# wwu98934/MuRCL

Measured on AMD Instinct MI355X. Metric: WSI-bags/sec pretrain step (ABMIL+NT-Xent) at N=2048,d=512, higher is better.
Workload: dtype bf16

## Files before the change

### include/murcl_amd.h

```cpp
#ifndef MURCL_AMD_H
#define MURCL_AMD_H
#include <stdint.h>
#ifdef __cplusplus
extern "C" {
#endif

typedef struct ihipStream_t* murcl_stream_t;

#define MURCL_F32 0
#define MURCL_BF16 1

#define MURCL_EPI_NONE 0
#define MURCL_EPI_BIAS 1
#define MURCL_EPI_BIAS_RELU 2
#define MURCL_EPI_MASK 3
#define MURCL_EPI_RANK1_MASK 4

int murcl_gemm_nt(const void* A, const void* B, void* C, int M, int N, int K, int lda, int ldb, int ldc,
                  int dtype_in, int dtype_out, int epilogue, const float* bias, const void* mask, int ldmask,
                  const float* rowscale, const float* rank1, int rows_per_bag, float* colsum_ws, int accumulate,
                  murcl_stream_t stream);

typedef struct murcl_tn_problem {
    const void* A; const void* B; float* C;
    const float* colsum_part; float* colsum_out;
    int M, N1, N2, lda, ldb, ldc, colsum_rows;
    int flags;
    float scale;
} murcl_tn_problem;
#define MURCL_TN_OVERWRITE 1
#define MURCL_TN_DEINTERLEAVE 2
#define MURCL_TN_SCALE 4
#define MURCL_TN_KIND_EMPTY 0
#define MURCL_TN_KIND_SMALL 1
#define MURCL_TN_KIND_SQUARE 2
#define MURCL_TN_KIND_PARTS 3
#define MURCL_TN_KIND_ATOMIC 4
#define MURCL_TN_KIND_WIDE 5
#define MURCL_TN_MAXG 4
long murcl_gemm_tn_plan(const murcl_tn_problem* probs, int n, int dtype, int* kinds);
int murcl_gemm_tn_grouped(const murcl_tn_problem* probs, int n, int dtype, float* ws, long ws_bytes, murcl_stream_t stream);

int murcl_panel_gemm_supported(int M, int N, int K, int epilogue, int rows_per_bag);
int murcl_panel_gemm_colsum_rows(int M, int N, int K, int epilogue);
int murcl_panel_gemm(const void* A, const void* W, void* C, int M, int N, int K, int epilogue, const float* bias,
                     void* bitmask_out, const void* bitmask_in, const float* rowscale, const float* rank1,
                     int rows_per_bag, float* colsum_out, int colsum_accumulate, float* colsum_ws ,
                     int walk_reverse, murcl_stream_t stream);
int murcl_panel_gemm_drop(const void* A, const void* W, void* C, int M, int N, int K, int epilogue, const float* bias,
                          void* bitmask_out, const void* bitmask_in, const float* rowscale, const float* rank1,
                          int rows_per_bag, float* colsum_out, int colsum_accumulate, float* colsum_ws, int walk_reverse,
                          float keep_p, unsigned long long seed_a, unsigned long long seed_b, murcl_stream_t stream);

int murcl_cu_budget(void);
int murcl_set_cu_budget(int cus);

int murcl_calib_copy(const void* src, void* dst, long bytes, murcl_stream_t stream);
int murcl_calib_mfma_bf16(float* out_256x512, int iters, murcl_stream_t stream);

int murcl_abmil_pool_workspace(int B, int N, int dtype, int* chunk_rows, int* n_chunks);
int murcl_abmil_pool_fwd(const void* H, const void* Wa, const float* ba, const float* wb, const float* bb,
                         float* scores, float* A, float* M, float* ml, float* part_ws, int B, int N, int L, int D,
                         int dtype, int exact_tanh, murcl_stream_t stream);
int murcl_abmil_pool_combine(const float* scores, const float* part_ws, float* A, float* M, float* ml, int B, int N,
                             int dtype, murcl_stream_t stream);
// ... 181 lines not shown
```

### murcl_amd/_lib.py

```python
import ctypes
import os

import torch

_HERE = os.path.dirname(os.path.abspath(__file__))
LIB_PATH = os.environ.get("MURCL_AMD_LIB") or os.path.join(_HERE, "libmurcl_amd.so")

F32, BF16 = 0, 1
EPI_NONE, EPI_BIAS, EPI_BIAS_RELU, EPI_MASK, EPI_RANK1_MASK = 0, 1, 2, 3, 4

_c = ctypes
_P, _I, _L, _F = _c.c_void_p, _c.c_int, _c.c_long, _c.c_float

SIGNATURES = {
    "murcl_gemm_nt": [_P, _P, _P, _I, _I, _I, _I, _I, _I, _I, _I, _I, _P, _P, _I, _P, _P, _I, _P, _I, _P],
    "murcl_gemm_tn_plan": [_P, _I, _I, _P],
    "murcl_gemm_tn_grouped": [_P, _I, _I, _P, _L, _P],
    "murcl_panel_gemm_colsum_rows": [_I, _I, _I, _I],
    "murcl_panel_gemm_supported": [_I, _I, _I, _I, _I],
    "murcl_panel_gemm": [_P, _P, _P, _I, _I, _I, _I, _P, _P, _P, _P, _P, _I, _P, _I, _P, _I, _P],
    "murcl_panel_gemm_drop": [_P, _P, _P, _I, _I, _I, _I, _P, _P, _P, _P, _P, _I, _P, _I, _P, _I, _F, ctypes.c_ulonglong, ctypes.c_ulonglong, _P],
    "murcl_cu_budget": [],
    "murcl_set_cu_budget": [_I],
    "murcl_calib_copy": [_P, _P, _L, _P],
# ... 69 lines not shown
    "murcl_gru_step_supported": [_I, _I, _I],
    "murcl_gru_step_fwd": [_P, _P, _I, _P, _P, _P, _P, _P, _P, _P, _I, _I, _P],
    "murcl_gru_step_bwd": [_P, _P, _P, _P, _P, _P, _P, _P, _P, _I, _I, _I, _I, _P],
    "murcl_ppo_act_workspace": [_I, _I, _I],
    "murcl_ppo_act": [_P, _I, _I, _I, _P, _P, _P, _F, _I, _P, _P, _P, _P, _P],
    "murcl_ppo_epoch_workspace": [_I, _I, _I, _I],
    "murcl_ppo_epoch": [_P, _P, _I, _I, _I, _P, _P, _P, _P, _I, _I, _L, _F, _F, _F, _P, _P, _P],
    "murcl_ppo_epoch_wt": [_P, _P, _P, _I, _I, _I, _P, _P, _P, _P, _I, _I, _L, _F, _F, _F, _P, _P, _P],
    "murcl_step_draws": [ctypes.c_ulonglong, _P, _L, _P, _L, _P, _P, _I, _I, _F, _P],
    "murcl_stack_lists": [_P, _I, _P],
    "murcl_add_lists": [_P, _I, _P],
    "murcl_cast_batch": [_P, _I, _I, _P],
    "murcl_cast_batch_flat": [_P, _P, _I, _I, _P],
    "murcl_cast_batch_flat_tick": [_P, _P, _I, _I, _P, _P],
    "murcl_relu_bitmask": [_P, _P, _I, _I, _I, _I, _P],
    "murcl_dropout_relu_bitmask": [_P, _P, _I, _I, _F, _F, ctypes.c_ulonglong, _I, _P],
    "murcl_adam_step": [_P, _P, _P, _P, _L, _F, _F, _F, _F, _F, _I, _I, _P],
    "murcl_adam_multi": [_P, _I, _F, _F, _F, _F, _I, _P],
    "murcl_adam_multi_live": [_P, _I, _F, _F, _F, _F, _I, _P, _P],
    "murcl_adam_multi_live_deferred": [_P, _I, _F, _F, _F, _F, _I, _P, _P],
    "murcl_replay_tick": [_P, _P],
    "murcl_sgd_step": [_P, _P, _P, _L, _F, _F, _I, _F, _I, _I, _P],
}
_RESTYPE = {"murcl_ntxent_workspace_bytes": _L, "murcl_ntxent_xchg_bytes": _L, "murcl_kmeans_workspace_bytes": _L, "murcl_ppo_act_workspace": _L, "murcl_gemm_tn_plan": _L,
            "murcl_ppo_epoch_workspace": _L}



class TnProblem(ctypes.Structure):
    _fields_ = [("A", _P), ("B", _P), ("C", _P), ("colsum_part", _P), ("colsum_out", _P),
                ("M", _I), ("N1", _I), ("N2", _I), ("lda", _I), ("ldb", _I), ("ldc", _I), ("colsum_rows", _I), ("flags", _I), ("scale", _F)]


TN_OVERWRITE, TN_DEINTERLEAVE, TN_SCALE = 1, 2, 4
TN_KIND_EMPTY, TN_KIND_SMALL, TN_KIND_SQUARE, TN_KIND_PARTS, TN_KIND_ATOMIC, TN_KIND_WIDE = 0, 1, 2, 3, 4, 5
TN_MAXG = 4


_lib = None


def lib():
    global _lib
    if _lib is None:
        if not os.path.exists(LIB_PATH):
            raise RuntimeError(
                f"{LIB_PATH} not found: build it with `python -m murcl_amd.build` "
                "(murcl_amd has no CPU/PyTorch fallback for its kernels)")
        L = ctypes.CDLL(LIB_PATH)
        for name, args in SIGNATURES.items():
            fn = getattr(L, name)
            fn.argtypes = args
            fn.restype = _RESTYPE.get(name, _I)
        _lib = L
    return _lib


def check(rc, what):
    if rc != 0:
        raise RuntimeError(f"murcl_amd: {what} failed with code {rc}")


def ptr(t):
    return None if t is None else t.data_ptr()


_raw_stream = getattr(torch._C, "_cuda_getCurrentRawStream", None)
# ... 15 lines not shown
```

### murcl_amd/csrc/gemm.hip

```cpp
#include "common.h"

enum { EPI_NONE = 0, EPI_BIAS = 1, EPI_BIAS_RELU = 2, EPI_MASK = 3, EPI_RANK1_MASK = 4 };

struct GemmEpi {
    const float* bias;
    const void* mask;
    int ldmask;
    const float* rowscale;
    const float* rank1;
    int rows_per_bag;
    float* colsum_ws;
    int accumulate;
};

template <typename T> struct Frag;
template <> struct Frag<bf16_t> { typedef bf16x8 type; };
template <> struct Frag<float> { typedef f32x4 type; };

template <typename T>
__device__ __forceinline__ f32x4 mma16(typename Frag<T>::type a, typename Frag<T>::type b, f32x4 c);
template <>
__device__ __forceinline__ f32x4 mma16<bf16_t>(bf16x8 a, bf16x8 b, f32x4 c) {
    return __builtin_amdgcn_mfma_f32_16x16x32_bf16(a, b, c, 0, 0, 0);
}
// ... 918 lines not shown
            __builtin_amdgcn_sched_group_barrier(0x008, NJ / 4, 0);
            __builtin_amdgcn_sched_group_barrier(0x100, 1, 0);
            __builtin_amdgcn_sched_group_barrier(0x008, NJ / 4, 0);
            __builtin_amdgcn_sched_group_barrier(0x100, 1, 0);
            __builtin_amdgcn_sched_group_barrier(0x008, NJ / 2, 0);
        }
        __builtin_amdgcn_sched_group_barrier(0x008, 2 * NJ, 0);
    }
    float* pt = part + (size_t)sp * N1 * N2;
    const int q4 = lane >> 4, r16 = lane & 15;
#pragma unroll
    for (int i = 0; i < 8; ++i)
#pragma unroll
        for (int j = 0; j < NJ; ++j) {
            const int n2 = n20 + wc * (16 * NJ) + j * 16 + r16;
#pragma unroll
            for (int r = 0; r < 4; ++r) {
                const int n1 = n10 + wr * 128 + i * 16 + 4 * q4 + r;
                pt[(size_t)n1 * N2 + n2] = acc[i][j][r];
            }
        }
}
struct TnReduceArgs {
    float* C[TN_MAXG];
    const float* cs_part[TN_MAXG];
    float* cs_out[TN_MAXG];
    long part_off[TN_MAXG], n4[TN_MAXG];
    int nsplit[TN_MAXG], N1[TN_MAXG], N2[TN_MAXG], ldc[TN_MAXG], cs_rows[TN_MAXG], flags[TN_MAXG];
    float scale[TN_MAXG];
    int blk0[TN_MAXG + 1];
    int cs_blk0[TN_MAXG + 1];
    int n;
};
__global__ __launch_bounds__(256) void tn_reduce_kernel(const float* __restrict__ ws, const TnReduceArgs ra) {
    int blk = blockIdx.x;
    if (blk >= ra.blk0[ra.n]) {
        blk -= ra.blk0[ra.n];
        int g = 0;
        while (g + 1 < ra.n && blk >= ra.cs_blk0[g + 1]) ++g;
        blk -= ra.cs_blk0[g];
        const float* __restrict__ cs_part = ra.cs_part[g];
        if (cs_part == nullptr) return;
        const int cs_rows = ra.cs_rows[g];
        __shared__ f32x4 red[256];
        const int cg = threadIdx.x & 15, rs = threadIdx.x >> 4;
        const long j = (long)blk * 16 + cg;
        const int ng = ra.N1[g] / 4;
        f32x4 b0 = {0, 0, 0, 0}, b1 = b0;
        if (j < ng) {
            const f32x4* q = (const f32x4*)cs_part + j;
            for (int r0 = 0; r0 < cs_rows; r0 += 256) {
                f32x4 v[16];
#pragma unroll
                for (int k = 0; k < 16; ++k) {
                    const int r = r0 + rs + 16 * k;
                    v[k] = r < cs_rows ? q[(size_t)r * ng] : f32x4{0, 0, 0, 0};
                }
#pragma unroll
                for (int k = 0; k < 16; k += 2) { b0 += v[k]; b1 += v[k + 1]; }
            }
        }
        red[threadIdx.x] = b0 + b1;
        __syncthreads();
        if (rs == 0 && j < ng) {
            f32x4 t = red[cg];
#pragma unroll
            for (int k = 1; k < 16; ++k) t += red[16 * k + cg];
            if (ra.flags[g] & MURCL_TN_SCALE) t *= ra.scale[g];
            f32x4* o = (f32x4*)ra.cs_out[g] + j;
            *o = (ra.flags[g] & MURCL_TN_OVERWRITE) ? t : *o + t;
        }
        return;
    }
    int g = 0;
    while (g + 1 < ra.n && blk >= ra.blk0[g + 1]) ++g;
    const long i = (long)(blk - ra.blk0[g]) * 256 + threadIdx.x;
    const long n4 = ra.n4[g];
    if (i >= n4) return;
    const int nsplit = ra.nsplit[g], N2 = ra.N2[g];
    const f32x4* p = (const f32x4*)(ws + ra.part_off[g]) + i;
    f32x4 a0 = {0, 0, 0, 0}, a1 = a0, a2 = a0, a3 = a0;
    int s = 0;
    for (; s + 3 < nsplit; s += 4) {
        const f32x4 v0 = p[(size_t)s * n4], v1 = p[(size_t)(s + 1) * n4], v2 = p[(size_t)(s + 2) * n4], v3 = p[(size_t)(s + 3) * n4];
        a0 += v0; a1 += v1; a2 += v2; a3 += v3;
    }
    for (; s < nsplit; ++s) a0 += p[(size_t)s * n4];
    f32x4 t = (a0 + a1) + (a2 + a3);
    const int fl = ra.flags[g];
    if (fl & MURCL_TN_SCALE) t *= ra.scale[g];
    const long e = i * 4, col = e % N2;
    long row = e / N2;
    if (fl & MURCL_TN_DEINTERLEAVE) row = ((row >> 4) & 1) * (ra.N1[g] >> 1) + (row >> 5) * 16 + (row & 15);
    f32x4* c = (f32x4*)(ra.C[g] + row * ra.ldc[g] + col);
    *c = (fl & MURCL_TN_OVERWRITE) ? t : *c + t;
}
static bool tn_sq_ok(int M, int N1, int N2, int ldc, int dtype) {
    return dtype == MURCL_DTYPE_BF16 && N1 % 256 == 0 && N2 % 256 == 0 && M >= 16384 && ldc % 4 == 0;
}
struct TnPlan { int sp[TN_MAXG], mps[TN_MAXG], tiles[TN_MAXG]; long part_off[TN_MAXG]; long ws_floats; int wgs; };
static bool tn_group_plan(int n, const int* M, const int* N1, const int* N2, TnPlan* pl, unsigned* map) {
    if (n < 1 || n > TN_MAXG) return false;
    long work = 0;
    int pairs = 0;
    for (int g = 0; g < n; ++g) {
        pl->tiles[g] = (N1[g] / 256) * (N2[g] / 256);
        if (pl->tiles[g] > murcl_cu_budget() / 8) return false;
        work += (long)pl->tiles[g] * M[g];
        pairs += pl->tiles[g];
    }
    const int cap = murcl_cu_budget();
    if (pairs > cap) return false;
    long R = ((work + cap - 1) / cap + 31) / 32 * 32;
    if (R < 8 * 32) R = 8 * 32;
    for (;; R += ((R >> 8) + 31) / 32 * 32) {
        int total = 0;
        for (int g = 0; g < n; ++g) {
            pl->sp[g] = (int)((M[g] + R - 1) / R);
            total += pl->sp[g] * pl->tiles[g];
        }
        if (total <= cap) { pl->wgs = total; break; }
    }
    long off = 0;
    for (int g = 0; g < n; ++g) {
        long mps = ((M[g] + pl->sp[g] - 1) / pl->sp[g] + 31) / 32 * 32;
        pl->mps[g] = (int)mps;
        pl->sp[g] = (int)((M[g] + mps - 1) / mps);
        pl->part_off[g] = off;
// ... 68 lines not shown
        if (mc & 15) {
            const int nz = (mp - mc) * 32;
            for (int i = tid; i < 2 * nz; i += 256) {
                const int which = i >= nz, j = which ? i - nz : i;
                *(float*)(ts_smem + (which ? slab_b : 0u) + (mc * 32 + j) * 4) = 0.f;
            }
            __syncthreads();
        }
        const char* la = ts_smem + aoff;
        const char* lb = ts_smem + slab_b + boff;
        for (int u = 0; u < mp / 16; ++u) {
            f32x4 a, b;
#pragma unroll
            for (int e = 0; e < 4; ++e) {
                a[e] = *(const float*)(la + (16 * u + 4 * e) * 128);
                b[e] = *(const float*)(lb + (16 * u + 4 * e) * 128);
            }
            if (u & 1) acc1 = mma16<float>(a, b, acc1); else acc0 = mma16<float>(a, b, acc0);
            if (do_cs) accs = mma16<float>(a, f32x4{1.f, 1.f, 1.f, 1.f}, accs);
        }
    }
    const int n2 = n20 + 16 * wn + r16;
#pragma unroll
    for (int r = 0; r < 4; ++r) {
        const int n1 = n10 + 16 * wm + 4 * q4 + r;
        if (n1 < N1 && n2 < N2) C[(size_t)n1 * ldc + n2] = cold[r] + (acc0[r] + acc1[r]);
        if (do_cs && r16 == 0 && n1 < N1) colsum_out[n1] = overwrite ? accs[r] : colsum_out[n1] + accs[r];
    }
}
struct TnSmallGroup {
    const float* A[4]; const float* B[4]; float* C[4]; float* cs[4];
    int M[4], N1[4], N2[4], lda[4], ldb[4], ldc[4], tile0[5], pass_rows, overwrite[4];
};
__global__ __launch_bounds__(256) void gemm_tn_small_group_kernel(const TnSmallGroup ga) {
    extern __shared__ __attribute__((aligned(16))) char ts_smem[];
    const int b = blockIdx.x;
    int g = 0;
#pragma unroll
    for (int i = 1; i < 4; ++i) g += (int)(b >= ga.tile0[i]);
    const int t = b - ga.tile0[g], t1 = (ga.N1[g] + TS_T - 1) / TS_T;
    tn_small_tile(ga.A[g], ga.B[g], ga.C[g], ga.M[g], ga.N1[g], ga.N2[g], ga.lda[g], ga.ldb[g], ga.ldc[g], ga.cs[g], t % t1, t / t1,
                  ts_smem, ga.pass_rows, ga.overwrite[g]);
}
static int tn_small_pass_rows(int M, long tiles) {
    int pr = TS_MAXM;
    if (tiles > 512 && M > 192) pr = ((M + 1) / 2 + 15) & ~15;
    pr = (pr + 15) & ~15;
    if (pr > TS_MAXM) pr = TS_MAXM;
    if (pr < 16) pr = 16;
    return pr;
}


static void tn_generic_plan(int M, int N1, int N2, int dtype, bool x3, int& splits, int& mps) {
    const int rows = dtype == MURCL_DTYPE_BF16 ? 64 : 32;
    const int t1 = (N1 + 127) / 128, t2 = (N2 + 127) / 128;
    if (M <= 8 * rows && (long)N1 * N2 >= (1L << 20)) {
        splits = 1;
    } else {
        const int target = (dtype == MURCL_DTYPE_F32 && !x3 && M >= 16384) ? 2 * murcl_cu_budget() : murcl_cu_budget();
        splits = (target + t1 * t2 - 1) / (t1 * t2);
        if (splits >= 8) splits = ((splits + 7) / 8) * 8;
        if (murcl_cu_budget() < 256 && splits >= 8)
            while (splits > 8 && splits * t1 * t2 > target) splits -= 8;
        while (splits > 8 && (long)(splits - 8) * rows * 4 >= M) splits -= 8;
        while (splits > 1 && splits < 8 && (long)(splits - 1) * rows * 4 >= M) --splits;
    }
    mps = (M + splits - 1) / splits;
    mps = ((mps + rows - 1) / rows) * rows;
    if ((long)mps * (splits - 1) >= M) splits = (M + mps - 1) / mps;
}

constexpr int TN_PARTS_MIN_M = 16384;
static_assert(TN_MAXG == MURCL_TN_MAXG, "include/murcl_amd.h");

typedef murcl_tn_problem TnProblem;
struct TnStep { int kind, splits, mps; long ws_bytes; };

static int tn_plan_one(const TnProblem& p, int dtype, TnStep& st) {
    st = TnStep{MURCL_TN_KIND_EMPTY, 0, 0, 0};
    if (p.M <= 0 || p.N1 <= 0 || p.N2 <= 0) return p.flags ? -1 : 0;
    if (p.colsum_part && (!p.colsum_out || p.colsum_rows <= 0 || p.N1 % 4)) return -1;
    const bool x3 = dtype == MURCL_DTYPE_F32X3;
    const int base = x3 ? MURCL_DTYPE_F32 : dtype;
    if (base != MURCL_DTYPE_F32 && base != MURCL_DTYPE_BF16) return -1;
    const int es = base == MURCL_DTYPE_BF16 ? 2 : 4, epc = 16 / es;
    if (p.N1 < epc || p.N2 < epc || p.N1 % epc || p.N2 % epc || (p.lda * es) % 16 || (p.ldb * es) % 16) return -1;
    TnPlan pl;
    if (tn_sq_ok(p.M, p.N1, p.N2, p.ldc, dtype) && tn_group_plan(1, &p.M, &p.N1, &p.N2, &pl, nullptr)) {
        st = TnStep{MURCL_TN_KIND_SQUARE, pl.sp[0], pl.mps[0], pl.ws_floats * 4};
        return p.flags && p.colsum_out && !p.colsum_part ? -1 : 0;
    }
    if (dtype == MURCL_DTYPE_BF16 && p.N1 % 256 == 0 && p.N2 % 128 == 0 && p.M >= 4096) {
        const int tiles = (p.N1 / 256) * (p.N2 / 128);
        int sp = (256 + tiles - 1) / tiles;
        sp = ((sp + 7) / 8) * 8;
        while (sp > 8 && (long)(sp - 8) * 64 * 4 >= p.M) sp -= 8;
        int mps = (p.M + sp - 1) / sp;
        mps = ((mps + 63) / 64) * 64;
        if ((long)mps * (sp - 1) >= p.M) sp = (p.M + mps - 1) / mps;
        st = TnStep{MURCL_TN_KIND_WIDE, sp, mps, 0};
        return p.flags ? -1 : 0;
    }
    if (dtype == MURCL_DTYPE_F32 && p.M <= TS_MAXM) {
        st = TnStep{MURCL_TN_KIND_SMALL, 1, p.M, 0};
        return (p.flags & ~MURCL_TN_OVERWRITE) || (p.flags && p.colsum_part) ? -1 : 0;
    }
    int splits, mps;
    tn_generic_plan(p.M, p.N1, p.N2, base, x3, splits, mps);
    if (p.M >= TN_PARTS_MIN_M && splits > 1 && (long)mps * (splits - 1) < p.M)
        st = TnStep{MURCL_TN_KIND_PARTS, splits, mps, (long)splits * ((long)p.N1 * p.N2 + p.N1) * 4};
    else
        st = TnStep{MURCL_TN_KIND_ATOMIC, splits, mps, 0};
    return p.flags ? -1 : 0;
}

enum { TN_EACH, TN_SMALL_GROUP, TN_SQ_GROUP };
static long tn_plan(const TnProblem* pr, int n, int dtype, int* kinds, int& form) {
    form = TN_EACH;
    bool small = n <= TN_MAXG, sq = n <= TN_MAXG;
    long ws = 0;
    int M[TN_MAXG], N1[TN_MAXG], N2[TN_MAXG];
    for (int g = 0; g < n; ++g) {
        TnStep st;
        if (tn_plan_one(pr[g], dtype, st)) return -1;
        if (kinds) kinds[g] = st.kind;
        small = small && st.kind == MURCL_TN_KIND_SMALL && !pr[g].colsum_part;
        sq = sq && st.kind == MURCL_TN_KIND_SQUARE;
        ws = st.ws_bytes > ws ? st.ws_bytes : ws;
        if (g < TN_MAXG) { M[g] = pr[g].M; N1[g] = pr[g].N1; N2[g] = pr[g].N2; }
    }
    if (n < 1) return 0;
    if (small) form = TN_SMALL_GROUP;
    TnPlan pl;
    if (sq && tn_group_plan(n, M, N1, N2, &pl, nullptr)) {
        form = TN_SQ_GROUP;
        ws = pl.ws_floats * 4;
    }
    return ws;
}

extern "C" long murcl_gemm_tn_plan(const TnProblem* pr, int n, int dtype, int* kinds) {
    int form;
    return tn_plan(pr, n, dtype, kinds, form);
}

static int tn_small_launch(const TnProblem* pr, int n, hipStream_t stream) {
    TnSmallGroup ga;
    int tiles = 0, mmax = 0;
    for (int g = 0; g < 4; ++g) {
        const TnProblem& p = pr[g < n ? g : 0];
        ga.A[g] = (const float*)p.A; ga.B[g] = (const float*)p.B; ga.C[g] = p.C; ga.cs[g] = p.colsum_out;
        ga.M[g] = p.M; ga.N1[g] = p.N1; ga.N2[g] = p.N2; ga.lda[g] = p.lda; ga.ldb[g] = p.ldb; ga.ldc[g] = p.ldc;
        ga.overwrite[g] = (p.flags & MURCL_TN_OVERWRITE) ? 1 : 0;
        ga.tile0[g] = tiles;
        if (g < n) {
            tiles += ((p.N1 + TS_T - 1) / TS_T) * ((p.N2 + TS_T - 1) / TS_T);
            if (p.M > mmax) mmax = p.M;
        }
    }
    for (int g = n; g < 5; ++g) ga.tile0[g] = tiles;
    ga.pass_rows = tn_small_pass_rows(mmax, tiles);
    const int mp = ((mmax < ga.pass_rows ? mmax : ga.pass_rows) + 15) & ~15;
    static MurclOncePerDevice once;
    if (once.first())
        hipFuncSetAttribute((const void*)gemm_tn_small_group_kernel, hipFuncAttributeMaxDynamicSharedMemorySize, 2 * TS_MAXM * 128);
    hipLaunchKernelGGL(gemm_tn_small_group_kernel, dim3(tiles), dim3(256), 2 * mp * 128, stream, ga);
    return MURCL_CHECK_LAUNCH();
}

static int tn_sq_launch(const TnProblem* pr, int n, int dtype, float* ws, hipStream_t stream) {
    int M[TN_MAXG], N1[TN_MAXG], N2[TN_MAXG];
    for (int g = 0; g < n; ++g) {
        M[g] = pr[g].M; N1[g] = pr[g].N1; N2[g] = pr[g].N2;
        if (pr[g].colsum_out && !pr[g].colsum_part) {
            const int rc = murcl_colsum(pr[g].A, pr[g].colsum_out, pr[g].M, pr[g].N1, pr[g].lda, dtype, 1, stream);
            if (rc) return rc;
        }
    }
    TnPlan pl;
    TnGroupArgs ga;
    if (!tn_group_plan(n, M, N1, N2, &pl, ga.map)) return -1;
    TnReduceArgs ra;
    ra.n = n;
    int blk = 0, csb = 0;
    for (int g = 0; g < TN_MAXG; ++g) {
        const int h = g < n ? g : 0;
        ga.A[g] = (const bf16_t*)pr[h].A; ga.B[g] = (const bf16_t*)pr[h].B;
        ga.M[g] = pr[h].M; ga.N1[g] = pr[h].N1; ga.N2[g] = pr[h].N2; ga.lda[g] = pr[h].lda; ga.ldb[g] = pr[h].ldb;
        ga.mps[g] = pl.mps[h]; ga.part_off[g] = pl.part_off[h];
        ra.C[g] = pr[h].C; ra.cs_part[g] = pr[h].colsum_part; ra.cs_out[g] = pr[h].colsum_part ? pr[h].colsum_out : nullptr;
        ra.cs_rows[g] = pr[h].colsum_rows;
        ra.part_off[g] = pl.part_off[h]; ra.n4[g] = (long)pr[h].N1 * pr[h].N2 / 4; ra.nsplit[g] = pl.sp[h];
        ra.N1[g] = pr[h].N1; ra.N2[g] = pr[h].N2; ra.ldc[g] = pr[h].ldc; ra.flags[g] = pr[h].flags; ra.scale[g] = pr[h].scale;
        if (g < n) {
            ra.blk0[g] = blk; blk += (int)((ra.n4[g] + 255) / 256);
            ra.cs_blk0[g] = csb; csb += pr[g].colsum_part ? (pr[g].N1 / 4 + 15) / 16 : 0;
        }
    }
    for (int g = n; g <= TN_MAXG; ++g) { ra.blk0[g] = blk; ra.cs_blk0[g] = csb; }
    auto k = gemm_tn_sq_kernel<TN_SQ_WAVES>;
    constexpr int LDS = TN_SQ_NSLOT * 32768;
    static MurclOncePerDevice once;
    if (once.first()) { hipFuncSetAttribute((const void*)k, hipFuncAttributeMaxDynamicSharedMemorySize, LDS); }
    hipLaunchKernelGGL(k, dim3(TN_MAXWG), dim3(64 * TN_SQ_WAVES), LDS, stream, ga, ws);
    int rc = MURCL_CHECK_LAUNCH();
    if (rc) return rc;
    hipLaunchKernelGGL(tn_reduce_kernel, dim3((unsigned)(blk + csb)), dim3(256), 0, stream, (const float*)ws, ra);
    return MURCL_CHECK_LAUNCH();
}

static int tn_launch_one(TnProblem p, int dtype, float* ws, hipStream_t stream) {
    TnStep st;
    tn_plan_one(p, dtype, st);
    if (st.kind == MURCL_TN_KIND_EMPTY) return 0;
    if (st.kind == MURCL_TN_KIND_SQUARE) return tn_sq_launch(&p, 1, dtype, ws, stream);
    if (p.colsum_part) {
        const int rc = murcl_colsum(p.colsum_part, p.colsum_out, p.colsum_rows, p.N1, p.N1, MURCL_DTYPE_F32, 1, stream);
        if (rc) return rc;
        p.colsum_out = nullptr;
    }
    if (st.kind == MURCL_TN_KIND_SMALL) return tn_small_launch(&p, 1, stream);
    const void *A = p.A, *B = p.B;
    float *C = p.C, *colsum_out = p.colsum_out;
    const int M = p.M, N1 = p.N1, N2 = p.N2, lda = p.lda, ldb = p.ldb, ldc = p.ldc, splits = st.splits, mps = st.mps;
    if (st.kind == MURCL_TN_KIND_WIDE) {
        if (colsum_out) {
            const int rc = murcl_colsum(A, colsum_out, M, N1, lda, dtype, 1, stream);
            if (rc) return rc;
        }
        auto k = gemm_tn_wide_kernel;
        constexpr int LDS = 3 * 49152;
        static MurclOncePerDevice once;
        if (once.first()) { hipFuncSetAttribute((const void*)k, hipFuncAttributeMaxDynamicSharedMemorySize, LDS); }
        hipLaunchKernelGGL(k, dim3((N1 / 256) * (N2 / 128) * splits), dim3(512), LDS, stream, (const bf16_t*)A, (const bf16_t*)B, C,
                           M, N1, N2, lda, ldb, ldc, mps, splits);
        return MURCL_CHECK_LAUNCH();
    }
    const bool x3 = dtype == MURCL_DTYPE_F32X3;
    float* part = st.kind == MURCL_TN_KIND_PARTS ? ws : nullptr;
    const int rows = dtype == MURCL_DTYPE_BF16 ? 64 : 32;
    const int t1 = (N1 + 127) / 128, t2 = (N2 + 127) / 128;
    dim3 grid(t1 * t2 * splits);
    const bool deep = (t1 * t2 * splits <= 256 || splits == 1) && mps > rows;
#define TN_LAUNCH(T, NS, X3)                                                                                        \
    {                                                                                                               \
        auto k = gemm_tn_kernel<T, NS, X3>;                                                                         \
        static MurclOncePerDevice once;                                                                                         \
        if (once.first()) { hipFuncSetAttribute((const void*)k, hipFuncAttributeMaxDynamicSharedMemorySize, NS * 32768); } \
        hipLaunchKernelGGL(k, grid, dim3(256), NS * 32768, stream, (const T*)A, (const T*)B, C, M, N1, N2, lda, ldb, ldc, mps, \
                           splits, colsum_out, part);                                                               \
    }
    if (dtype == MURCL_DTYPE_BF16) {
        if (deep) TN_LAUNCH(bf16_t, 4, false) else TN_LAUNCH(bf16_t, 2, false)
    } else if (x3) {
        if (deep) TN_LAUNCH(float, 4, true) else TN_LAUNCH(float, 2, true)
    } else {
        if (deep) TN_LAUNCH(float, 4, false) else TN_LAUNCH(float, 2, false)
    }
#undef TN_LAUNCH
    if (part) {
        const int rc = MURCL_CHECK_LAUNCH();
        if (rc) return rc;
        const long n = (long)N1 * N2 + (colsum_out ? N1 : 0);
        hipLaunchKernelGGL(tn_split_reduce_kernel, dim3((unsigned)((n + 31) / 32)), dim3(256), 0, stream, part, C, colsum_out, N1, N2,
                           ldc, splits);
    }
    return MURCL_CHECK_LAUNCH();
}

extern "C" int murcl_gemm_tn_grouped(const TnProblem* pr, int n, int dtype, float* ws, long ws_bytes, hipStream_t stream) {
    int form;
    const long need = tn_plan(pr, n, dtype, nullptr, form);
    if (need < 0 || (need > 0 && (!ws || ws_bytes < need))) return -1;
    if (form == TN_SMALL_GROUP) return tn_small_launch(pr, n, stream);
    if (form == TN_SQ_GROUP) return tn_sq_launch(pr, n, dtype, ws, stream);
    for (int g = 0; g < n; ++g) {
        const int rc = tn_launch_one(pr[g], dtype, ws, stream);
        if (rc) return rc;
    }
    return 0;
}
```

### murcl_amd/functional.py

```python
import math

import torch

from . import ops


def _flat2(x):
    return x.reshape(-1, x.shape[-1])


_DIRECT = False


def set_direct_grad(flag):
    global _DIRECT
    _DIRECT = bool(flag)


_MILESTONE = None
_STREAM_A = 4
_FUSED_GATE = True
_GATE_U = True
_FUSED_FC_DROP = True
_FUSED_INST = True
_DSMIL_REASSOC = True
_DSMIL_ONEPASS = True
_DSMIL_QV = True
_DSMIL_X3 = True
_GROUP_WGRAD = True
_FOLD_BIAS = True
_FRAG_WEIGHTS = True


def _frag_specs(w1, w2, w3, wa, T):
    return [(w1, False, T, "frag"), (w2, False, T, "frag"), (w3, False, T, "frag"), (wa, False, T, "frag"),
            (wa, True, T), (w3, True, T, "frag"), (w2, True, T, "frag")]


_OVERLAP_BUDGET = None


def set_overlap_cu_budget(cus):
    global _OVERLAP_BUDGET
    _OVERLAP_BUDGET = None if cus is None else int(cus)


class _overlap_budget:

    def __enter__(self):
        self.prev = None
        if _OVERLAP_BUDGET is not None:
            self.prev = ops.cu_budget()
            ops.set_cu_budget(min(self.prev, _OVERLAP_BUDGET))
        return self

    def __exit__(self, *exc):
        if self.prev is not None:
            ops.set_cu_budget(self.prev)
        return False


def set_grad_milestone(callback):
    global _MILESTONE
    _MILESTONE = callback
# ... 73 lines not shown
def _wgrad_group(items):
    probs = []
    for dy, x, w, b, parts in items:
        if _direct(w):
            probs.append((dy, x, w.grad, b.grad.view(-1) if parts is not None else None, parts))
            _touch(w)
            if parts is not None:
                _touch(b)
        else:
            assert parts is None
            probs.append((dy, x, None, None, None))
    Cs = ops.gemm_tn_grouped(probs, fresh=True)
    return [None if _direct(it[2]) else C for it, C in zip(items, Cs)]


_DEFERRED = None
_DEFER_ON = True


class deferred_wgrads:
    def __enter__(self):
        global _DEFERRED
        self.prev, _DEFERRED = _DEFERRED, ({} if _DEFER_ON else None)
        return self

    def __exit__(self, *exc):
        global _DEFERRED
        queue, _DEFERRED = _DEFERRED, self.prev
        if exc[0] is None and queue:
            _flush(queue)
        return False


def _flush(queue):
    probs = []
    for w, b, dys, xs in queue.values():
        dy = dys[0] if len(dys) == 1 else torch.cat(dys, 0)
        x = xs[0] if len(xs) == 1 else torch.cat(xs, 0)
        probs.append((dy, x, w.grad, b.grad.view(-1) if b is not None else None, None))
    queue.clear()
    for i in range(0, len(probs), 4):
        ops.gemm_tn_grouped(probs[i:i + 4])


def flush_deferred():
    if _DEFERRED:
        _flush(_DEFERRED)


def _defer(dy, x, w, b):
    if _DEFERRED is None or not _direct(w) or (b is not None and not _direct(b)):
        return False
    ent = _DEFERRED.get(id(w))
    if ent is None:
        ent = _DEFERRED[id(w)] = (w, b, [], [])
    elif (ent[1] is None) != (b is None):
        return False
    ent[2].append(dy)
    ent[3].append(x)
    _touch(w, b)
    return True


def _wbgrad(dy, x, w, b):
    if _defer(dy, x, w, b):
        return None, None
    if _direct(w) and _direct(b):
        ops.gemm_tn(dy, x, out=w.grad, colsum_into=b.grad.view(-1))
        _touch(w, b)
        return None, None
    return _wgrad(dy, x, w), _bgrad(dy, b)


def _bgrad(dy, b):
    if _direct(b):
# ... 155 lines not shown
        if m3 is not None:
            dT, dba, dwb, dbb = ops.abmil_pool_bwd(h3.view(B, N, L), wac, ba, wb, scores, ml, M, dM, into=into_k2, frag=wfrag)
        else:
            dT, dba, dwb, dbb, A = ops.abmil_pool_bwd(h3.view(B, N, L), wac, ba, wb, scores, ml, M, dM, into=into_k2, want_A=True,
                                                      frag=wfrag)
        dwa = _wgrad(dT, h3, wa)
        if direct_k2:
            _touch(ba, wb, bb)
            _final(wa, ba, wb, bb, wd, bd)
        if m3 is not None:
            def into(b):
                if _direct(b):
                    _touch(b)
                    return b.grad.view(-1)
                return None
            fold = lambda w, b: _FOLD_BIAS and _direct(w) and _direct(b)
            f3, f2, f1 = fold(w3, b3), fold(w2, b2), fold(w1, b1)
            grouped = _GROUP_WGRAD and _MILESTONE is None
            dz3, _, db3 = ops.panel_gemm(dT, wat, ops.PG_RANK1_MASK, bitmask=m3, rowscale=scores.view(-1), bias=ml, rank1=dM,
                                         rows_per_bag=N, colsum=True, colsum_into=None if f3 else into(b3), colsum_defer=f3,
                                         frag=False)
            if not grouped:
                dw3 = _wgrad(dz3, h2, w3, b3, db3 if f3 else None)
                _final(w3, b3)
            dz2, _, db2 = ops.panel_gemm(dz3, w3t, ops.PG_MASK, bitmask=m2, colsum=True,
                                         colsum_into=None if f2 else into(b2), colsum_defer=f2, frag=wfrag)
            if not grouped:
                dw2 = _wgrad(dz2, h1, w2, b2, db2 if f2 else None)
                _final(w2, b2)
            dz1, _, db1 = ops.panel_gemm(dz2, w2t, ops.PG_MASK, bitmask=m1, colsum=True,
                                         colsum_into=None if f1 else into(b1), colsum_defer=f1, frag=wfrag)
            budget_scope.__exit__()
            if grouped:
                dw3, dw2, dw1 = _wgrad_group([(dz3, h2, w3, b3, db3 if f3 else None), (dz2, h1, w2, b2, db2 if f2 else None),
                                              (dz1, x2, w1, b1, db1 if f1 else None)])
                _final(w3, b3, w2, b2, w1, b1)
            db3, db2 = None if f3 else db3, None if f2 else db2
            if grouped:
                db1 = None if f1 else db1
        else:
            dz3, ws = ops.gemm_nt(dT, wat, epi=ops.EPI_RANK1_MASK, mask=h3, rowscale=A.view(-1),
                                  rank1=dM, rows_per_bag=N, colsum=True)
            db3 = _bgrad(ws, b3)
            dw3 = _wgrad(dz3, h2, w3)
            _final(w3, b3)
            dz2, ws = ops.gemm_nt(dz3, w3t, epi=ops.EPI_MASK, mask=h2, colsum=True)
            db2 = _bgrad(ws, b2)
            dw2 = _wgrad(dz2, h1, w2)
            _final(w2, b2)
            dz1, ws = ops.gemm_nt(dz2, w2t, epi=ops.EPI_MASK, mask=h1, colsum=True)
            db1 = _bgrad(ws, b1)
            budget_scope.__exit__()
        if m3 is not None and grouped:
            pass
        elif m3 is not None and f1:
            dw1, db1 = _wgrad(dz1, x2, w1, b1, db1), None
        else:
            dw1 = _wgrad(dz1, x2, w1)
        dx = None
        if need_dx:
            dx = ops.gemm_nt(dz1, ops.transpose_cast(w1, T)).view(B, N, d)
        if direct_k2:
            dba = dwb = dbb = None
        else:
            dba, dwb, dbb = _pgrad(dba, ba), _pgrad(dwb.reshape(1, -1), wb), _pgrad(dbb, bb)
        return dx, dw1, db1, dw2, db2, dw3, db3, dwa, dba, dwb, dbb, dwd, dbd

    @staticmethod
# ... 861 lines not shown
```

### murcl_amd/ops.py

```python
import ctypes
import math

import torch

from . import _lib
from ._lib import BF16, F32, EPI_BIAS, EPI_BIAS_RELU, EPI_MASK, EPI_NONE, EPI_RANK1_MASK, check, dt, ptr, stream

_TORCH_DT = {F32: torch.float32, BF16: torch.bfloat16}
_EPI_NAME = {EPI_NONE: "NONE", EPI_BIAS: "BIAS", EPI_BIAS_RELU: "BIAS_RELU", EPI_MASK: "MASK", EPI_RANK1_MASK: "RANK1_MASK"}
_DT_NAME = {torch.float32: "f32", torch.bfloat16: "bf16"}


class KernelTimers:

    def __init__(self, only=None, every=1, pool=0):
        self.only, self.every, self.records, self._seen = only, max(1, int(every)), {}, {}
        self._pool = [torch.cuda.Event(enable_timing=True) for _ in range(int(pool))]

    def event(self):
        return self._pool.pop() if self._pool else torch.cuda.Event(enable_timing=True)

    def span(self, key, work=None):
        if self.only is not None and key not in self.only:
            return _NULL
# ... 202 lines not shown
            check(_lib.lib().murcl_panel_gemm_drop(ptr(A), ptr(W), ptr(C), M, N, K, epi, ptr(bias), ptr(bm), ptr(bitmask),
                                                   ptr(rowscale), ptr(rank1), rows_per_bag,
                                                   ptr(colsum_into if colsum_into is not None else cs),
                                                   int(colsum_into is not None), ptr(ws), int(reverse) | (2 if stream_a else 0) | wfrag,
                                                   drop.keep_p, drop.seed, 0, stream()), "panel_gemm(drop)")
        else:
            check(_lib.lib().murcl_panel_gemm(ptr(A), ptr(W), ptr(C), M, N, K, epi, ptr(bias), ptr(bm), ptr(bitmask),
                                              ptr(rowscale), ptr(rank1), rows_per_bag,
                                              ptr(colsum_into if colsum_into is not None else cs),
                                              int(colsum_into is not None), ptr(ws), int(reverse) | (2 if stream_a else 0) | wfrag, stream()),
                  "panel_gemm")
    if colsum_defer:
        return C, bm, (ws, _lib.lib().murcl_panel_gemm_colsum_rows(M, N, K, epi))
    return C, bm, cs


def relu_bitmask(x):
    _need_cuda(x)
    x = _c(x)
    M, N = x.shape
    bits = torch.empty((M, N // 8), dtype=torch.uint8, device=x.device)
    check(_lib.lib().murcl_relu_bitmask(ptr(x), ptr(bits), M, N, N, dt(x), stream()), "relu_bitmask")
    return bits


_TN_NAME = {_lib.TN_KIND_SQUARE: "gemm_tn_sq", _lib.TN_KIND_WIDE: "gemm_tn_wide"}
_CODE_NAME = {F32: "f32", BF16: "bf16", F32X3: "f32x3"}


def gemm_tn_plan(problems, code):
    n = len(problems)
    arr, kinds = (_lib.TnProblem * n)(), (ctypes.c_int * n)()
    for g, (A, B, _, ci, cp, opts) in enumerate(problems):
        assert A.dtype == B.dtype == problems[0][0].dtype and A.shape[0] == B.shape[0]
        (M, N1), N2 = A.shape, B.shape[1]
        flags, scale = 0, 1.0
        if opts and opts.get("scale") is not None:
            flags, scale = flags | _lib.TN_SCALE, float(opts["scale"])
        if opts and opts.get("deinterleave"):
            flags |= _lib.TN_DEINTERLEAVE
        if opts and opts.get("overwrite"):
            flags |= _lib.TN_OVERWRITE
        assert ci is None or (ci.dtype == torch.float32 and ci.is_contiguous() and ci.numel() == N1)
        arr[g] = _lib.TnProblem(ptr(A), ptr(B), None, ptr(cp[0]) if cp else None, ptr(ci), M, N1, N2, N1, N2, N2, cp[1] if cp else 0,
                                flags, scale)
    return arr, _lib.lib().murcl_gemm_tn_plan(arr, n, code, kinds), list(kinds)


def _tn_sq_group(kinds):
    return 1 < len(kinds) <= _lib.TN_MAXG and all(k == _lib.TN_KIND_SQUARE for k in kinds)


def _tn_run(problems, code, plan, write):
    arr, wsb, kinds = plan
    if wsb < 0:
        raise RuntimeError(f"murcl_amd: murcl_gemm_tn_plan rejects {[(tuple(p[0].shape), tuple(p[1].shape)) for p in problems]} ({wsb})")
    Cs, written = [], False
    for g, (A, B, out, *_) in enumerate(problems):
        N1, N2 = A.shape[1], B.shape[1]
        if out is None:
            written = write(kinds[g], problems[g])
            out = (torch.empty if written else torch.zeros)((N1, N2), dtype=torch.float32, device=A.device)
            if written:
                arr[g].flags |= _lib.TN_OVERWRITE
        assert out.dtype == torch.float32 and out.is_contiguous() and tuple(out.shape) == (N1, N2)
        arr[g].C = ptr(out)
        Cs.append(out)
    ws = torch.empty((wsb // 4,), dtype=torch.float32, device=Cs[0].device) if wsb else None
    if _tn_sq_group(kinds):
        key = f"gemm_tn_sq_grouped{len(kinds)}<bf16>"
    elif all(k == _lib.TN_KIND_SMALL for k in kinds) and (len(kinds) > 1 or written):
        key = None
    else:
        key = "+".join(sorted({_TN_NAME.get(k, "gemm_tn") for k in kinds})) + f"<{_CODE_NAME[code]}>"
    span = _span(lambda: (key, dict(flops=sum(2.0 * p[0].shape[0] * p[0].shape[1] * p[1].shape[1] for p in problems),
                                    bytes=sum(p[0].shape[0] * (p[0].shape[1] + p[1].shape[1]) * p[0].element_size()
                                              + p[0].shape[1] * p[1].shape[1] * 4 for p in problems)))) if key else _NULL
    with span:
        check(_lib.lib().murcl_gemm_tn_grouped(arr, len(problems), code, ptr(ws), wsb, stream()), "gemm_tn_grouped")
    return Cs


def gemm_tn_with_colsum(A, B):
    _need_cuda(A, B)
    A, B = _c(A), _c(B)
    cs = torch.empty((A.shape[1],), dtype=torch.float32, device=A.device)
    probs = [(A, B, None, cs, None, None)]
    plan = gemm_tn_plan(probs, dt(A))
    if plan[1] < 0 or plan[2][0] != _lib.TN_KIND_SMALL:
        return gemm_tn(A, B), colsum(A)
    return _tn_run(probs, dt(A), plan, lambda k, p: True)[0], cs


def gemm_tn(A, B, *, out=None, colsum_into=None, colsum_parts=None, x3=False):
    _need_cuda(A, B)
    A, B = _c(A), _c(B)
    M, N1 = A.shape
    N2 = B.shape[1]
    assert B.shape[0] == M and A.dtype == B.dtype
    epc = 4 if A.dtype == torch.float32 else 8
    if colsum_parts is not None and (colsum_into is None or N1 % 4):
        raise ValueError("colsum_parts needs colsum_into and N1 % 4 == 0")
    if N1 % epc:
        res = gemm_tn(pad_cols(A, ((N1 + epc - 1) // epc) * epc), B)[:N1]
        if colsum_into is not None:
            colsum(A, out=colsum_into, accumulate=True)
        if out is None:
            return res.contiguous()
        if out.is_contiguous() and out.dtype == torch.float32:
            return axpby(out, res, 1.0, 1.0, out=out)
        return out.add_(res)
    fresh = out is None and colsum_into is None and not x3
    code = F32X3 if (x3 and A.dtype == torch.float32 and M >= 4096) else dt(A)
    probs = [(A, B, out, colsum_into, colsum_parts, None)]
    return _tn_run(probs, code, gemm_tn_plan(probs, code), lambda k, p: fresh and k == _lib.TN_KIND_SMALL)[0]


def gemm_tn_grouped(problems, fresh=False):
    problems = [(_c(p[0]), _c(p[1])) + tuple(p[2:]) + (None,) * (6 - len(p)) for p in problems]
    _need_cuda(*(t for p in problems for t in p[:2]))
    if any(p[0].shape[1] % (16 // p[0].element_size()) for p in problems):
        assert all(p[5] is None for p in problems), "scale / deinterleave / overwrite need the grouped launch"
        return [gemm_tn(A, B, out=out, colsum_into=ci, colsum_parts=cp) for A, B, out, ci, cp, _ in problems]
    code = dt(problems[0][0])
    plan = gemm_tn_plan(problems, code)
    sq_group = _tn_sq_group(plan[2])
    return _tn_run(problems, code, plan, lambda k, p: (k == _lib.TN_KIND_SMALL and p[3] is None)
                   or (k == _lib.TN_KIND_SQUARE and fresh and sq_group))


def gemm_tn_grouped_ok(problems):
    problems = [tuple(p) + (None,) * (6 - len(p)) for p in problems]
    _, wsb, kinds = gemm_tn_plan(problems, dt(problems[0][0]))
    return wsb >= 0 and _tn_sq_group(kinds)


def cu_budget():
    return _lib.lib().murcl_cu_budget()


def set_cu_budget(cus):
    return _lib.lib().murcl_set_cu_budget(int(cus))


def pool_chunks(B, N, dtype_code):
    cr, nc = ctypes.c_int(), ctypes.c_int()
    _lib.lib().murcl_abmil_pool_workspace(B, N, dtype_code, ctypes.byref(cr), ctypes.byref(nc))
    return cr.value, nc.value


def _pool_work(B, N, L, D, es):
    return dict(flops=B * (2.0 * N * L * D + 2.0 * N * D + 2.0 * N * L), bytes=B * (N * L * es + N * 4 + L * 4) + L * D * es)


def abmil_pool_partials(H, Wa, ba, wb, bb, exact_tanh=None, scores=None, frag=None):
    _need_cuda(H, Wa)
    wfrag = 2 if (is_frag(Wa) if frag is None else frag) else 0
    H, Wa = _c(H), (Wa if wfrag else _c(Wa))
    B, N, L = H.shape
    D = Wa.shape[0]
    if exact_tanh is None:
# ... 1033 lines not shown
```

Before: 44820.

## Fold deferred small f32 head wgrads into the square-group TN reduce launch

Adds an F32_IN flag so a grouped TN GEMM can mix bf16 square problems with f32 small problems. When the MLP wgrad group is deferred, the small head weight-gradient GEMMs are run inside the same epilogue kernel that performs the split-K reduction of the square group, instead of as separate launches. The aim is to cut kernel launches and tail idle time in the backward pass. The cost is more complex planning and the small tiles sharing a kernel with reduce blocks, with LDS sized for the larger of the two.

```diff
diff --git a/include/murcl_amd.h b/include/murcl_amd.h
--- a/include/murcl_amd.h
+++ b/include/murcl_amd.h
@@ -31,6 +31,7 @@
 #define MURCL_TN_OVERWRITE 1
 #define MURCL_TN_DEINTERLEAVE 2
 #define MURCL_TN_SCALE 4
+#define MURCL_TN_F32_IN 8
 #define MURCL_TN_KIND_EMPTY 0
 #define MURCL_TN_KIND_SMALL 1
 #define MURCL_TN_KIND_SQUARE 2
diff --git a/murcl_amd/_lib.py b/murcl_amd/_lib.py
--- a/murcl_amd/_lib.py
+++ b/murcl_amd/_lib.py
@@ -125,7 +125,7 @@
                 ("M", _I), ("N1", _I), ("N2", _I), ("lda", _I), ("ldb", _I), ("ldc", _I), ("colsum_rows", _I), ("flags", _I), ("scale", _F)]
 
 
-TN_OVERWRITE, TN_DEINTERLEAVE, TN_SCALE = 1, 2, 4
+TN_OVERWRITE, TN_DEINTERLEAVE, TN_SCALE, TN_F32_IN = 1, 2, 4, 8
 TN_KIND_EMPTY, TN_KIND_SMALL, TN_KIND_SQUARE, TN_KIND_PARTS, TN_KIND_ATOMIC, TN_KIND_WIDE = 0, 1, 2, 3, 4, 5
 TN_MAXG = 4
 
diff --git a/murcl_amd/csrc/gemm.hip b/murcl_amd/csrc/gemm.hip
--- a/murcl_amd/csrc/gemm.hip
+++ b/murcl_amd/csrc/gemm.hip
@@ -974,8 +974,7 @@
     int cs_blk0[TN_MAXG + 1];
     int n;
 };
-__global__ __launch_bounds__(256) void tn_reduce_kernel(const float* __restrict__ ws, const TnReduceArgs ra) {
-    int blk = blockIdx.x;
+__device__ __forceinline__ void tn_reduce_block(const float* __restrict__ ws, const TnReduceArgs& ra, int blk, f32x4* red) {
     if (blk >= ra.blk0[ra.n]) {
         blk -= ra.blk0[ra.n];
         int g = 0;
@@ -984,7 +983,6 @@
         const float* __restrict__ cs_part = ra.cs_part[g];
         if (cs_part == nullptr) return;
         const int cs_rows = ra.cs_rows[g];
-        __shared__ f32x4 red[256];
         const int cg = threadIdx.x & 15, rs = threadIdx.x >> 4;
         const long j = (long)blk * 16 + cg;
         const int ng = ra.N1[g] / 4;
@@ -1036,6 +1034,10 @@
     if (fl & MURCL_TN_DEINTERLEAVE) row = ((row >> 4) & 1) * (ra.N1[g] >> 1) + (row >> 5) * 16 + (row & 15);
     f32x4* c = (f32x4*)(ra.C[g] + row * ra.ldc[g] + col);
     *c = (fl & MURCL_TN_OVERWRITE) ? t : *c + t;
+}
+__global__ __launch_bounds__(256) void tn_reduce_kernel(const float* __restrict__ ws, const TnReduceArgs ra) {
+    __shared__ f32x4 red[256];
+    tn_reduce_block(ws, ra, blockIdx.x, red);
 }
 static bool tn_sq_ok(int M, int N1, int N2, int ldc, int dtype) {
     return dtype == MURCL_DTYPE_BF16 && N1 % 256 == 0 && N2 % 256 == 0 && M >= 16384 && ldc % 4 == 0;
@@ -1170,15 +1172,23 @@
     const float* A[4]; const float* B[4]; float* C[4]; float* cs[4];
     int M[4], N1[4], N2[4], lda[4], ldb[4], ldc[4], tile0[5], pass_rows, overwrite[4];
 };
-__global__ __launch_bounds__(256) void gemm_tn_small_group_kernel(const TnSmallGroup ga) {
-    extern __shared__ __attribute__((aligned(16))) char ts_smem[];
-    const int b = blockIdx.x;
+__device__ __forceinline__ void tn_small_block(const TnSmallGroup& ga, int b, char* ts_smem) {
     int g = 0;
 #pragma unroll
     for (int i = 1; i < 4; ++i) g += (int)(b >= ga.tile0[i]);
     const int t = b - ga.tile0[g], t1 = (ga.N1[g] + TS_T - 1) / TS_T;
     tn_small_tile(ga.A[g], ga.B[g], ga.C[g], ga.M[g], ga.N1[g], ga.N2[g], ga.lda[g], ga.ldb[g], ga.ldc[g], ga.cs[g], t % t1, t / t1,
                   ts_smem, ga.pass_rows, ga.overwrite[g]);
+}
+__global__ __launch_bounds__(256) void gemm_tn_small_group_kernel(const TnSmallGroup ga) {
+    extern __shared__ __attribute__((aligned(16))) char ts_smem[];
+    tn_small_block(ga, blockIdx.x, ts_smem);
+}
+__global__ __launch_bounds__(256) void tn_epilogue_kernel(const float* __restrict__ ws, const TnReduceArgs ra, const TnSmallGroup sg) {
+    extern __shared__ __attribute__((aligned(16))) char ts_smem[];
+    const int ns = sg.tile0[4];
+    if ((int)blockIdx.x < ns) tn_small_block(sg, blockIdx.x, ts_smem);
+    else tn_reduce_block(ws, ra, (int)blockIdx.x - ns, (f32x4*)ts_smem);
 }
 static int tn_small_pass_rows(int M, long tiles) {
     int pr = TS_MAXM;
@@ -1215,8 +1225,13 @@
 typedef murcl_tn_problem TnProblem;
 struct TnStep { int kind, splits, mps; long ws_bytes; };
 
-static int tn_plan_one(const TnProblem& p, int dtype, TnStep& st) {
+static int tn_plan_one(TnProblem p, int dtype, TnStep& st) {
     st = TnStep{MURCL_TN_KIND_EMPTY, 0, 0, 0};
+    if (p.flags & MURCL_TN_F32_IN) {
+        if (dtype != MURCL_DTYPE_BF16) return -1;
+        dtype = MURCL_DTYPE_F32;
+        p.flags &= ~MURCL_TN_F32_IN;
+    }
     if (p.M <= 0 || p.N1 <= 0 || p.N2 <= 0) return p.flags ? -1 : 0;
     if (p.colsum_part && (!p.colsum_out || p.colsum_rows <= 0 || p.N1 % 4)) return -1;
     const bool x3 = dtype == MURCL_DTYPE_F32X3;
@@ -1253,10 +1268,12 @@
     return p.flags ? -1 : 0;
 }
 
-enum { TN_EACH, TN_SMALL_GROUP, TN_SQ_GROUP };
-static long tn_plan(const TnProblem* pr, int n, int dtype, int* kinds, int& form) {
+enum { TN_EACH, TN_SMALL_GROUP, TN_SQ_GROUP, TN_EPILOGUE };
+static long tn_plan(const TnProblem* pr, int n, int dtype, int* kinds, int& form, int* nsq = nullptr) {
     form = TN_EACH;
+    if (nsq) *nsq = 0;
     bool small = n <= TN_MAXG, sq = n <= TN_MAXG;
+    int lead = 0, tail = 0;
     long ws = 0;
     int M[TN_MAXG], N1[TN_MAXG], N2[TN_MAXG];
     for (int g = 0; g < n; ++g) {
@@ -1265,6 +1282,8 @@
         if (kinds) kinds[g] = st.kind;
         small = small && st.kind == MURCL_TN_KIND_SMALL && !pr[g].colsum_part;
         sq = sq && st.kind == MURCL_TN_KIND_SQUARE;
+        if (st.kind == MURCL_TN_KIND_SQUARE && lead == g && lead < TN_MAXG) ++lead;
+        else if (st.kind == MURCL_TN_KIND_SMALL && !pr[g].colsum_part && (pr[g].flags & MURCL_TN_F32_IN) && lead && tail < 4) ++tail;
         ws = st.ws_bytes > ws ? st.ws_bytes : ws;
         if (g < TN_MAXG) { M[g] = pr[g].M; N1[g] = pr[g].N1; N2[g] = pr[g].N2; }
     }
@@ -1274,6 +1293,10 @@
     if (sq && tn_group_plan(n, M, N1, N2, &pl, nullptr)) {
         form = TN_SQ_GROUP;
         ws = pl.ws_floats * 4;
+    } else if (tail && lead + tail == n && tn_group_plan(lead, M, N1, N2, &pl, nullptr)) {
+        form = TN_EPILOGUE;
+        ws = pl.ws_floats * 4;
+        if (nsq) *nsq = lead;
     }
     return ws;
 }
@@ -1283,8 +1306,7 @@
     return tn_plan(pr, n, dtype, kinds, form);
 }
 
-static int tn_small_launch(const TnProblem* pr, int n, hipStream_t stream) {
-    TnSmallGroup ga;
+static int tn_small_args(const TnProblem* pr, int n, TnSmallGroup& ga, int& lds) {
     int tiles = 0, mmax = 0;
     for (int g = 0; g < 4; ++g) {
         const TnProblem& p = pr[g < n ? g : 0];
@@ -1300,14 +1322,22 @@
     for (int g = n; g < 5; ++g) ga.tile0[g] = tiles;
     ga.pass_rows = tn_small_pass_rows(mmax, tiles);
     const int mp = ((mmax < ga.pass_rows ? mmax : ga.pass_rows) + 15) & ~15;
+    lds = 2 * mp * 128;
+    return tiles;
+}
+static int tn_small_launch(const TnProblem* pr, int n, hipStream_t stream) {
+    TnSmallGroup ga;
+    int lds;
+    const int tiles = tn_small_args(pr, n, ga, lds);
     static MurclOncePerDevice once;
     if (once.first())
         hipFuncSetAttribute((const void*)gemm_tn_small_group_kernel, hipFuncAttributeMaxDynamicSharedMemorySize, 2 * TS_MAXM * 128);
-    hipLaunchKernelGGL(gemm_tn_small_group_kernel, dim3(tiles), dim3(256), 2 * mp * 128, stream, ga);
+    hipLaunchKernelGGL(gemm_tn_small_group_kernel, dim3(tiles), dim3(256), lds, stream, ga);
     return MURCL_CHECK_LAUNCH();
 }
 
-static int tn_sq_launch(const TnProblem* pr, int n, int dtype, float* ws, hipStream_t stream) {
+static int tn_sq_launch(const TnProblem* pr, int n, int dtype, float* ws, hipStream_t stream, const TnProblem* small = nullptr,
+                        int n_small = 0) {
     int M[TN_MAXG], N1[TN_MAXG], N2[TN_MAXG];
     for (int g = 0; g < n; ++g) {
         M[g] = pr[g].M; N1[g] = pr[g].N1; N2[g] = pr[g].N2;
@@ -1344,6 +1374,17 @@
     hipLaunchKernelGGL(k, dim3(TN_MAXWG), dim3(64 * TN_SQ_WAVES), LDS, stream, ga, ws);
     int rc = MURCL_CHECK_LAUNCH();
     if (rc) return rc;
+    if (n_small > 0) {
+        TnSmallGroup sg;
+        int lds;
+        const int tiles = tn_small_args(small, n_small, sg, lds);
+        lds = lds > (int)(256 * sizeof(f32x4)) ? lds : (int)(256 * sizeof(f32x4));
+        static MurclOncePerDevice once_e;
+        if (once_e.first())
+            hipFuncSetAttribute((const void*)tn_epilogue_kernel, hipFuncAttributeMaxDynamicSharedMemorySize, 2 * TS_MAXM * 128);
+        hipLaunchKernelGGL(tn_epilogue_kernel, dim3((unsigned)(tiles + blk + csb)), dim3(256), lds, stream, (const float*)ws, ra, sg);
+        return MURCL_CHECK_LAUNCH();
+    }
     hipLaunchKernelGGL(tn_reduce_kernel, dim3((unsigned)(blk + csb)), dim3(256), 0, stream, (const float*)ws, ra);
     return MURCL_CHECK_LAUNCH();
 }
@@ -1408,13 +1449,17 @@
 }
 
 extern "C" int murcl_gemm_tn_grouped(const TnProblem* pr, int n, int dtype, float* ws, long ws_bytes, hipStream_t stream) {
-    int form;
-    const long need = tn_plan(pr, n, dtype, nullptr, form);
+    int form, nsq;
+    const long need = tn_plan(pr, n, dtype, nullptr, form, &nsq);
     if (need < 0 || (need > 0 && (!ws || ws_bytes < need))) return -1;
     if (form == TN_SMALL_GROUP) return tn_small_launch(pr, n, stream);
     if (form == TN_SQ_GROUP) return tn_sq_launch(pr, n, dtype, ws, stream);
+    if (form == TN_EPILOGUE) return tn_sq_launch(pr, nsq, dtype, ws, stream, pr + nsq, n - nsq);
     for (int g = 0; g < n; ++g) {
-        const int rc = tn_launch_one(pr[g], dtype, ws, stream);
+        TnProblem p = pr[g];
+        const int dt = (p.flags & MURCL_TN_F32_IN) ? MURCL_DTYPE_F32 : dtype;
+        p.flags &= ~MURCL_TN_F32_IN;
+        const int rc = tn_launch_one(p, dt, ws, stream);
         if (rc) return rc;
     }
     return 0;
diff --git a/murcl_amd/functional.py b/murcl_amd/functional.py
--- a/murcl_amd/functional.py
+++ b/murcl_amd/functional.py
@@ -30,6 +30,7 @@
 _GROUP_WGRAD = True
 _FOLD_BIAS = True
 _FRAG_WEIGHTS = True
+_FOLD_EPILOGUE = True
 
 
 def _frag_specs(w1, w2, w3, wa, T):
@@ -169,15 +170,37 @@
         return False
 
 
+_GROUPS = "wgrad groups"
+
+
 def _flush(queue):
+    groups = queue.pop(_GROUPS, [])
     probs = []
     for w, b, dys, xs in queue.values():
         dy = dys[0] if len(dys) == 1 else torch.cat(dys, 0)
         x = xs[0] if len(xs) == 1 else torch.cat(xs, 0)
         probs.append((dy, x, w.grad, b.grad.view(-1) if b is not None else None, None))
     queue.clear()
-    for i in range(0, len(probs), 4):
+    i = 0
+    for grp in groups:
+        if i == 0 and probs and ops.gemm_tn_epilogue(grp, probs[:4]):
+            i = 4
+        else:
+            ops.gemm_tn_grouped(grp, fresh=True)
+    for i in range(i, len(probs), 4):
         ops.gemm_tn_grouped(probs[i:i + 4])
+
+
+def _defer_group(items):
+    if not _FOLD_EPILOGUE or _DEFERRED is None or not all(_direct(w) and (parts is None or _direct(b)) for _, _, w, b, parts in items):
+        return False
+    _DEFERRED.setdefault(_GROUPS, []).append(
+        [(dy, x, w.grad, b.grad.view(-1) if parts is not None else None, parts) for dy, x, w, b, parts in items])
+    for _, _, w, b, parts in items:
+        _touch(w)
+        if parts is not None:
+            _touch(b)
+    return True
 
 
 def flush_deferred():
@@ -399,8 +422,10 @@
                                          colsum_into=None if f1 else into(b1), colsum_defer=f1, frag=wfrag)
             budget_scope.__exit__()
             if grouped:
-                dw3, dw2, dw1 = _wgrad_group([(dz3, h2, w3, b3, db3 if f3 else None), (dz2, h1, w2, b2, db2 if f2 else None),
-                                              (dz1, x2, w1, b1, db1 if f1 else None)])
+                items = [(dz3, h2, w3, b3, db3 if f3 else None), (dz2, h1, w2, b2, db2 if f2 else None), (dz1, x2, w1, b1, db1 if f1 else None)]
+                dw3 = dw2 = dw1 = None
+                if not _defer_group(items):
+                    dw3, dw2, dw1 = _wgrad_group(items)
                 _final(w3, b3, w2, b2, w1, b1)
             db3, db2 = None if f3 else db3, None if f2 else db2
             if grouped:
diff --git a/murcl_amd/ops.py b/murcl_amd/ops.py
--- a/murcl_amd/ops.py
+++ b/murcl_amd/ops.py
@@ -258,9 +258,10 @@
     n = len(problems)
     arr, kinds = (_lib.TnProblem * n)(), (ctypes.c_int * n)()
     for g, (A, B, _, ci, cp, opts) in enumerate(problems):
-        assert A.dtype == B.dtype == problems[0][0].dtype and A.shape[0] == B.shape[0]
+        f32_in = code == BF16 and A.dtype == torch.float32
+        assert A.dtype == B.dtype and (f32_in or A.dtype == problems[0][0].dtype) and A.shape[0] == B.shape[0]
         (M, N1), N2 = A.shape, B.shape[1]
-        flags, scale = 0, 1.0
+        flags, scale = _lib.TN_F32_IN if f32_in else 0, 1.0
         if opts and opts.get("scale") is not None:
             flags, scale = flags | _lib.TN_SCALE, float(opts["scale"])
         if opts and opts.get("deinterleave"):
@@ -295,6 +296,9 @@
     ws = torch.empty((wsb // 4,), dtype=torch.float32, device=Cs[0].device) if wsb else None
     if _tn_sq_group(kinds):
         key = f"gemm_tn_sq_grouped{len(kinds)}<bf16>"
+    elif any(arr[g].flags & _lib.TN_F32_IN for g in range(len(kinds))):
+        nsq = sum(k == _lib.TN_KIND_SQUARE for k in kinds)
+        key = f"gemm_tn_sq_grouped{nsq}+small{len(kinds) - nsq}<bf16>"
     elif all(k == _lib.TN_KIND_SMALL for k in kinds) and (len(kinds) > 1 or written):
         key = None
     else:
@@ -353,6 +357,21 @@
     sq_group = _tn_sq_group(plan[2])
     return _tn_run(problems, code, plan, lambda k, p: (k == _lib.TN_KIND_SMALL and p[3] is None)
                    or (k == _lib.TN_KIND_SQUARE and fresh and sq_group))
+
+
+def gemm_tn_epilogue(group, heads):
+    group = [tuple(p) + (None,) * (6 - len(p)) for p in group]
+    heads = [tuple(p) + (None,) * (6 - len(p)) for p in heads]
+    if not (1 <= len(heads) <= 4 and all(p[2] is not None for p in group + heads) and all(p[4] is None for p in heads)
+            and all(p[0].dtype == torch.float32 for p in heads)):
+        return False
+    probs = [(_c(p[0]), _c(p[1])) + tuple(p[2:]) for p in group + heads]
+    plan = gemm_tn_plan(probs, BF16)
+    if plan[1] < 0 or not _tn_sq_group(plan[2][:len(group)]) or plan[2][len(group):] != [_lib.TN_KIND_SMALL] * len(heads):
+        return False
+    _need_cuda(*(t for p in probs for t in p[:2]))
+    _tn_run(probs, BF16, plan, lambda k, p: False)
+    return True
 
 
 def gemm_tn_grouped_ok(problems):
```

Result: no change. 44860 (median of 4 runs) (+0.1%).
